# imaranresearch/LAMMPS-SPHERHARM

Measured on AMD Instinct MI355X. Metric: contact_pairs_per_sec, higher is better.
Workload: dtype f64; 1 GPU; BASELINE configs[1]: 100000 particles/GPU, 1 SH shape(s) L_max=6, dense packed bed (jittered HCP, spacing 1.9 mean radii), n_q=16 (Q=512 nodes/pair), pair_coeff kn=1000 exponent=1.25 (overlap volume + force + torque), inputs resident in HBM; particles_per_gpu=100000, lmax=6, nq=16, rule=sharp, backend=none, half_list_pairs_rank0=579574, contact_pairs_rank0=579574, touching_pairs_rank0=502600, contact_pairs_all_ranks=579574

## Files before the change

lammps-spherharm_amd/csrc/contact_kernel_azimuth.hpp:

```cpp
#pragma once
#include "contact_plan.hpp"
#include "jpoly.hpp"
#include "pair_params.hpp"
#include "pair_rotate.hpp"
#include "ring_tables.hpp"
#include "wave_ops.hpp"

namespace shp {


template <int L, bool NEEDV, int WPP = 1, bool SPEC = false>
__global__ void __launch_bounds__(64 * kMaxWavesPerBlock, SHP_JMIN_WAVES(L, NEEDV, WPP)) pair_contact_azimuth_kernel(const PairParams P)
{
  static_assert(L >= 0, "per-azimuth kernels: compiled orders only");
  constexpr int LJ = L;
  static_assert(!SPEC || (PairSpec<LJ>::nq > 0 && PairSpec<LJ>::wpp == WPP),
                "specialised instances: the orders PairSpec names");
  static_assert(WPP == 1 || WPP == 2, "one or two waves per pair");
  extern __shared__ __attribute__((aligned(16))) unsigned char smem_raw[];
  int lane = threadIdx.x & 63;
  const int wib = __builtin_amdgcn_readfirstlane((int)(threadIdx.x >> 6));
  const int w = P.slot0 + ((WPP == 2) ? (int)blockIdx.x : __builtin_amdgcn_readfirstlane((int)(blockIdx.x * P.waves_per_block)) + wib);
  const int half = (WPP == 2) ? wib : 0;
  const int tid = lane + 64 * half;
  constexpr int NT = 64 * WPP;
  if (w >= P.npairs) return;
  const int LL = L;
  typedef PairSpec<L> Spec;
  const int nq = SPEC ? Spec::nq : P.nq;
  const int P_ring_rows = SPEC ? Spec::rr : P.ring_rows;
  const int P_qcap = SPEC ? Spec::qc : P.qcap;
  constexpr bool P1S = SHP_SURFACE_PHASE1(L, NEEDV, WPP);
  constexpr bool CARRY = !P1S && SHP_CARRY_NODE(L, WPP);
  WaveLdsLayout W = (WPP == 2) ? pair_lds_layout2(LL, P_ring_rows, nq, P_qcap)
                               : wave_lds_layout(LL, P_ring_rows, false, nq, P_qcap);
  if constexpr (WPP == 2) {
    W.qri += half * W.qstride;
    W.qrj += half * W.qstride;
    W.qp += half * W.qstride;
    W.park += half * W.qstride;
  }
  typedef __attribute__((address_space(3))) unsigned char lds_byte_t;
  const unsigned wave_off = (WPP == 2) ? 0u : (unsigned)(wib * P.wave_lds_bytes);
  const unsigned wave_abs = __builtin_amdgcn_readfirstlane((unsigned)(size_t)(lds_byte_t*)smem_raw + wave_off);
#define WAVE_LDS() ((double*)(lds_byte_t*)(size_t)launder_s32(wave_abs))
  double* lw = WAVE_LDS();

  __builtin_amdgcn_s_setprio(3);
  const int* rid = P.rec_i + 4 * (size_t)w;
  constexpr int NSL = ((L + 1) * (L + 1) + NT - 1) / NT;
  double vi[NSL], vj[NSL];
  JPolyPre<LJ> pre;
  const double recv = P.rec[(size_t)kRecStride * w + (lane < kRecUsed ? lane : 0)];
  {
    constexpr int ns = (L + 1) * (L + 1);
#pragma unroll
    for (int t = 0; t < NSL; ++t) {
      const int e = tid + NT * t;
      const int ec = e < ns ? e : 0;
      if constexpr (rot_tiled(L)) {
        const int l = (int)__builtin_amdgcn_sqrtf((float)ec + 0.5f);
        const double* tile = P.rot + (size_t)((2 * w) >> 6) * rot_tile_doubles(L);
        const unsigned at = 64u * (unsigned)(l * l) + (unsigned)((2 * w) & 63) * (unsigned)(2 * l + 1) + (unsigned)(ec - l * l);
        vi[t] = tile[at];
        vj[t] = tile[at + (unsigned)(2 * l + 1)];
      } else {
        const size_t at = (size_t)(2 * w) * rot_row_doubles(L) + ec;
        vi[t] = P.rot[at];
        vj[t] = P.rot[at + rot_row_doubles(L)];
      }
    }
    pre.fetch(P, lane, nq);
  }
  double glt_first = 0.0, glw_first = 0.0;
  glw_first = P.glw[tid < nq ? tid : 0];
  if constexpr (L <= 8 && WPP == 1) {
    const int nr0 = P_ring_rows < nq ? P_ring_rows : nq;
    const int lg0 = ring_poly_map(nr0, L + 1, 64);
    const int kr = lg0 >= 1 ? (lane >> lg0) : lane / (L + 1);
    glt_first = P.glt[kr < nr0 ? kr : nr0 - 1];
  }
  const int status = rid[0];
  if (status == 0) return;
  double s_rho = 0.0, s_rj = 0.0, s_rj2 = 0.0, s_rho2 = 0.0, s_pj = 0.0, s_tol1 = 0.0, s_tol3 = 0.0, s_tiny = 0.0;
  {
    const cdptr rs = launder_uniform(P.rec + (size_t)kRecStride * w);
    s_rho = rs[FR_RHO];
    s_rj = rs[FR_RJ];
    s_rj2 = rs[FR_RJ2];
    s_rho2 = rs[FR_RHO2];
    s_pj = rs[FR_JPJ];
    s_tol1 = rs[FR_JTOL1];
    s_tol3 = rs[FR_JTOL3];
    s_tiny = rs[FR_JTINY];
  }
  const bool centre_in_bj = rid[3] != 0;
  if ((tid >= 12 && tid < 30) || (tid >= 36 && tid < kRecUsed)) lw[frj(tid)] = recv;
  if constexpr (L <= 8 && WPP == 1) lw[W.stash + lane] = glt_first;
#pragma unroll
  for (int t = 0; t < NSL; ++t)
    if (tid + NT * t < (LJ + 1) * (LJ + 1)) {
      lw[W.v0 + tid + NT * t] = vj[t];
      lw[W.v0i + tid + NT * t] = vi[t];
    }
  pair_sync<WPP>();
#if defined(SHP_ABL) && SHP_ABL == 1
  asm volatile("" ::"v"(lw[lane & 31]));
  return;
#endif
  jpoly_build<LJ, WPP>(P, lw, W, lane, nq, pre, glw_first, half);
#if defined(SHP_ABL) && SHP_ABL == 4
  asm volatile("" ::"v"(lw[W.pi + lane]));
  return;
#endif

  const double* fr = WAVE_LDS();

  bool centre_inside = false;
  if (NEEDV && centre_in_bj) {
    const double rho = fr[frj(FR_RHO)];
    const double rj = jpoly_eval<LJ>(fr + W.gh, -1.0, 0.0);
    centre_inside = (rho - rj <= 0.0);
  }

  const int npsi = 2 * nq;
  const unsigned magic = ((1u << 24) + (unsigned)npsi - 1u) / (unsigned)npsi;
  const int per_ring = nq / WPP;
  const unsigned magicr = ((1u << 24) + (unsigned)per_ring - 1u) / (unsigned)per_ring;
  const int nslabs = (nq * per_ring + 63) >> 6;
  const int rowlen = 4 * (LL + 1);

  {
    const int kend0 = (P_ring_rows < nq) ? P_ring_rows : nq;
    cap_frame_rings_poly<LJ, WPP>(P, WAVE_LDS(), W, lane, tid, 0, kend0, fr[frj(FR_HW)], fr[frj(FR_HM)], L <= 8 && WPP == 1);
  }
  bool first_group = true;
  double aV = 0.0, aS0 = 0.0, aS1 = 0.0, aS2 = 0.0, aT0 = 0.0, aT1 = 0.0, aT2 = 0.0;
#if defined(SHP_ABL) && SHP_ABL == 3
  int qhead = 0;
#endif
  int qcount = 0, slab = 0;

  while (slab < nslabs) {
  const int sfirst = slab;
  const int k0 = (int)(((unsigned)(sfirst << 6) * magicr) >> 24);
  const int kend = (k0 + P_ring_rows < nq) ? k0 + P_ring_rows : nq;
  const int slab_end = (kend == nq) ? nslabs : ((kend * per_ring) >> 6);
  if (slab_end <= slab) return;
  __builtin_amdgcn_s_setprio(3);
  {
    double* lr = WAVE_LDS();
    if (!first_group) {
      double* park = lr + W.park + lane;
      park[0] = aT2; park[64] = NEEDV ? aV : aS0;
      if constexpr (WPP == 2) __syncthreads();
      cap_frame_rings_poly<LJ, WPP>(P, lr, W, lane, tid, k0, kend - k0, lr[frj(FR_HW)], lr[frj(FR_HM)], false);
      park = WAVE_LDS() + W.park + lane;
      aT2 = park[0];
      if (NEEDV) aV = park[64]; else aS0 = park[64];
      wave_lds_sync();
    }
    first_group = false;
#if defined(SHP_ABL) && SHP_ABL == 2
    asm volatile("" ::"v"(lr[W.ring + lane]));
    return;
#endif
  }

  auto surface = [&](const double ri, const double rmu, const double rpsi, const double c, const double s, const double mu,
                     const double sig, const double isig, const double omi) __attribute__((always_inline)) {
    const double rad = ri * fma(ri, sig, rmu * sig * mu);
    const double tan_ = ri * rpsi * isig;
    const double A0 = fma(rad, c, tan_ * s);
    const double A1 = fma(rad, s, -tan_ * c);
    const double A2 = ri * fma(ri, mu, -(sig * sig) * rmu);
    aS0 = fma(omi, A0, aS0);
    aS1 = fma(omi, A1, aS1);
    aS2 = fma(omi, A2, aS2);
    const double wr = omi * ri;
    const double u0 = sig * c, u1 = sig * s;
    aT0 = fma(wr, u1 * A2 - mu * A1, aT0);
    aT1 = fma(wr, mu * A0 - u0 * A2, aT1);
    aT2 = fma(wr, u0 * A1 - u1 * A0, aT2);
  };
  auto phase2 = [&](auto dir_c, const int dp, const double dri, const double drj, const unsigned long long mdir)
                    __attribute__((always_inline)) {
    constexpr bool DIR = decltype(dir_c)::value;
    (void)dp; (void)dri; (void)drj; (void)mdir;
    wave_lds_sync();
    fr = WAVE_LDS();
    const int cnt = DIR ? 64 : (qcount < 64 ? qcount : 64);
    const bool active = DIR ? lane_of(mdir) : lane < cnt;
    if constexpr (!DIR) qcount -= cnt;
    const int e = DIR ? 0 : qcount + min(lane, cnt - 1);
#ifdef SHP_STATS
    if (lane == 0) atomicAdd(&P.dbg[4], 1ULL);
    if (active) atomicAdd(&P.dbg[7], 1ULL);
#endif
    int p;
    double ri;
    if constexpr (DIR) {
      p = dp;
      ri = dri;
    } else {
      p = ((const unsigned short*)(fr + W.qp))[e];
      ri = fr[W.qri + e];
    }
    int k = (int)(umul_sel<true>((unsigned)p, magic) >> 24);
    int l = p - mul_sel<true>(k, npsi);
    double omi = active ? fr[frj(FR_WSC)] * fr[W.glw + mul_sel<true>(k, jpoly_row(LJ))] : 0.0;
    const double omi3 = omi * (1.0 / 3.0);
    double c1 = 0.0, s1 = 0.0;
    if constexpr (!P1S) {
      c1 = P.cpsi[l];
      s1 = P.spsi[l];
    }
    double mu, sig;
    {
      const double* row = fr + W.ring + (k - k0) * rowlen;
      mu = row[1];
      sig = row[3];
    }

    double rin = 0.0;
    if (NEEDV) {
      const double rj0 = DIR ? drj : fr[W.qrj + e];
      double uj0, uj1;
      const int ghrow_ = W.gh + mul_sel<true>(l >= nq ? l - nq : l, jpoly_row(LJ));
      uj0 = mu;
      uj1 = (l >= nq) ? -sig : sig;
      double lo = 0.0, hi = ri, lam, xa = ri, ga, xb = ri, gb;
      {
        double bp, s2i;
        {
          const double rho = s_rho;
          bp = mu * rho;
          const double q0 = fma(ri, uj0, -rho), q1 = ri * uj1;
          s2i = fma(q0, q0, q1 * q1);
        }
        const double rho2l = s_rho2;
        if (!centre_in_bj) lo = bp - sqrt_nr1<true>(fma(bp, bp, -s_pj));
        lam = bp - sqrt_nr1<true>(fma(bp, bp, -(rho2l - rj0 * rj0)));
        if (!(lam > lo && lam < hi)) lam = 0.5 * (lo + hi);
        ga = gb = sqrt_nr1<true>(s2i) - rj0;
      }
      unsigned jrow_addr = wave_abs + 8u * (unsigned)ghrow_;
      unsigned long long mact;
      mact = centre_inside ? 0ULL : (DIR ? mdir : (cnt >= 64 ? ~0ULL : ((1ULL << cnt) - 1ULL)));
      auto iterate = [&](double& xa, double& ga, const double xb, const double gb, const double lam, double& gc,
                         const bool have3) __attribute__((always_inline)) {
#ifdef SHP_STATS
        if (lane == 0) atomicAdd(&P.dbg[5], 1ULL);
        if (lane_of(mact)) atomicAdd(&P.dbg[6], 1ULL);
#endif
        double y0, y1, ss2;
        y0 = fma(lam, uj0, -s_rho);
        y1 = lam * uj1;
        ss2 = fma(y0, y0, y1 * y1);
        const bool z0 = !(ss2 > 0.0);
        const double iv = rsqrt_nr1(ss2);
        double rj;
        jrow_addr = launder_u32(jrow_addr);
        rj = jpoly_eval<LJ>((const double*)(lds_byte_t*)(size_t)jrow_addr, y0 * iv, y1 * iv);
        const double Rjl = s_rj;
        double gl = ss2 * iv - rj;
        if (wave_any(z0)) {
          asm volatile("; rare: a point on x_j");
          gl = z0 ? -Rjl : gl;
        }
        {
          const bool pos = gl >= 0.0;
          lo = pos ? lam : lo;
          hi = pos ? hi : lam;
          const double dbl = gb - gl;
          double ext;
          if (!have3) {
            ext = fma(gl * (lam - xb), rcp_nr1(dbl), lam);
          } else {
            const double dab = ga - gb, dal = ga - gl;
            const double num = fma(xa * gb, gl * dbl, fma(lam * ga, gb * dab, -(xb * ga) * (gl * dal)));
            ext = num * rcp_nr1(dab * dal * dbl);
          }
          const bool inb = ext > lo && ext < hi;
          const bool accept = fabs(gl) <= (have3 ? s_tol3 : s_tol1);
          const bool tiny = hi - lo <= s_tiny;
          double res = ext, nxt = ext;
          unsigned long long mstop = wave_ballot(accept);
          if (mask_any(mact & (wave_ballot(tiny) | ~(wave_ballot(ext > lo) & wave_ballot(ext < hi))))) {
#ifdef SHP_STATS
            if (lane == 0) atomicAdd(&P.dbg[8], 1ULL);
#endif
            double sec = ext, e2 = ext;
            if (have3) {
              const double s2 = fma(gl * (lam - xb), rcp_nr1(dbl), lam);
              const bool fin0 = fabs(ext) <= 1e300;
              sec = (!fin0 || !inb) ? s2 : ext;
              e2 = fin0 ? ext : s2;
            }
            const double mid = 0.5 * (lo + hi);
            double n2 = (e2 > lo && e2 < hi) ? e2 : sec;
            n2 = (n2 > lo && n2 < hi) ? n2 : mid;
            const double accv = (fabs(e2) <= 1e300) ? fmin(fmax(e2, lo), hi) : lam;
            res = accept ? accv : (tiny ? mid : n2);
            nxt = n2;
            mstop |= wave_ballot(tiny);
          }
          rin = lane_of(mact) ? res : rin;
          mact &= ~mstop;
          gc = gl;
          xa = nxt;
        }
      };
      double gl0 = 0.0;
      if constexpr (SHP_PEEL(L)) {
      do {
        if (!mask_any(mact)) break;
        iterate(xa, ga, xb, gb, lam, gl0, false);
        if (!mask_any(mact)) break;
        iterate(xb, gb, lam, gl0, xa, ga, true);
        if (!mask_any(mact)) break;
        iterate(lam, gl0, xa, ga, xb, gb, true);
        for (int it = 3; it < 60; it = __builtin_amdgcn_readfirstlane(it + 3)) {
          if (!mask_any(mact)) break;
          iterate(xa, ga, xb, gb, lam, gl0, true);
          if (!mask_any(mact)) break;
          iterate(xb, gb, lam, gl0, xa, ga, true);
          if (!mask_any(mact)) break;
          iterate(lam, gl0, xa, ga, xb, gb, true);
        }
      } while (false);
      } else {
      for (int it = 0; it < 60; it = __builtin_amdgcn_readfirstlane(it + 3)) {
        if (!mask_any(mact)) break;
        iterate(xa, ga, xb, gb, lam, gl0, it >= 1);
        if (!mask_any(mact)) break;
        iterate(xb, gb, lam, gl0, xa, ga, true);
        if (!mask_any(mact)) break;
        iterate(lam, gl0, xa, ga, xb, gb, true);
      }
      }
      if constexpr (P1S) {
        if constexpr (!DIR) ri = fr[W.qri + (int)launder_u32((unsigned)e)];
        const double dv3 = ri * ri * ri - rin * rin * rin;
        aV = fma(omi3, dv3, aV);
      } else {
        auto ri_again = [&]() __attribute__((always_inline)) {
          const int lrow = l >= nq ? l - nq : l;
          const double* tgd = jpoly_trig_sep(LJ) ? fr + W.tr + 2 * lrow : fr + W.gh + mul_sel<true>(lrow, jpoly_row(LJ)) + jpoly_trig(LJ);
          double cd = 1.0, sd = 0.0;
          if constexpr (LJ >= 1) {
            const v2d csd = lds2(tgd);
            const double sgd = (l >= nq) ? -1.0 : 1.0;
            cd = sgd * csd[0];
            sd = sgd * csd[1];
          }
          return ring_value<LJ>(fr + W.ring + (k - k0) * rowlen, cd, sd);
        };
        if constexpr (!CARRY) {
          if constexpr (!DIR) {
            const int e2 = (int)launder_u32((unsigned)e);
            ri = fr[W.qri + e2];
            p = ((const unsigned short*)(fr + W.qp))[e2];
          }
          p = (int)launder_u32((unsigned)p);
          k = (int)(umul_sel<true>((unsigned)p, magic) >> 24);
          l = p - mul_sel<true>(k, npsi);
          omi = active ? fr[frj(FR_WSC)] * fr[W.glw + mul_sel<true>(k, jpoly_row(LJ))] : 0.0;
          const double* row = fr + W.ring + (k - k0) * rowlen;
          mu = row[1];
          sig = row[3];
          if constexpr (DIR) ri = ri_again();
        } else {
          if constexpr (DIR) {
            ri = ri_again();
          } else {
            const int e2 = (int)launder_u32((unsigned)e);
            ri = fr[W.qri + e2];
          }
        }
        const double dv3 = ri * ri * ri - rin * rin * rin;
        aV = fma(omi * (1.0 / 3.0), dv3, aV);
      }
    }

#if !(defined(SHP_ABL) && SHP_ABL == 6)
    if constexpr (!P1S) {
      fr = WAVE_LDS();
      double rmu, rpsi;
      const double sg = (l >= nq) ? -1.0 : 1.0;
      const int lrow = l >= nq ? l - nq : l;
      const double* tg = jpoly_trig_sep(LJ) ? fr + W.tr + 2 * lrow : fr + W.gh + mul_sel<true>(lrow, jpoly_row(LJ)) + jpoly_trig(LJ);
      if constexpr (LJ >= 1) {
        const v2d cs1 = lds2(tg);
        c1 = sg * cs1[0];
        s1 = sg * cs1[1];
      }
      ring_grad_rec<LJ>(fr + W.ring + (k - k0) * rowlen, c1, s1, rmu, rpsi);
      surface(ri, rmu, rpsi, c1, s1, mu, sig, rcp_nr1(sig), omi);
    }
#endif
    wave_lds_sync();
  };
  __builtin_amdgcn_s_setprio(0);
  for (;;) {
#define SHP_PUSH(m_, pn, rin_, rjn_)                                                                                  \
    {                                                                                                                  \
      if (m_ != 0ULL) {                                                                                                \
        if (lane_of(m_)) {                                                                                             \
          const int pos_ = qcount + (int)__builtin_amdgcn_mbcnt_hi((unsigned)(m_ >> 32),                               \
                                                    __builtin_amdgcn_mbcnt_lo((unsigned)m_, 0u));                      \
          double* lq_ = WAVE_LDS();                                                                                     \
          ((unsigned short*)(lq_ + W.qp))[pos_] = (unsigned short)(pn);                                                \
          lq_[W.qri + pos_] = (rin_);                                                                                  \
          lq_[W.qrj + pos_] = (rjn_);                                                                                  \
        }                                                                                                              \
        qcount += __builtin_popcountll(m_);                                                                            \
      }                                                                                                                \
    }
    while (qcount < 64 && slab < slab_end) {
      fr = WAVE_LDS();
      const int pp = (slab << 6) + lane;
      const int ppc = min(pp, nq * per_ring - 1);
      const int k = (int)(umul_sel<true>((unsigned)ppc, magicr) >> 24);
      const int l = ppc - mul_sel<true>(k, per_ring) + half * per_ring;
      const double* row = fr + W.ring + (k - k0) * rowlen;
      const v2d r01 = lds2(row);
      const double mu = r01[1], sig = row[3];
      const double* gr = fr + W.gh + mul_sel<true>(l, jpoly_row(LJ));
      double ria, rib;
      {
        double c1 = 1.0, s1 = 0.0, unused0, unused1;
        if constexpr (LJ >= 1) {
          const v2d cs1 = lds2(jpoly_trig_sep(LJ) ? fr + W.tr + 2 * l : gr + jpoly_trig(LJ));
          c1 = cs1[0];
          s1 = cs1[1];
        }
        ring_pair_rec<LJ, false>(row, r01[0], c1, s1, ria, rib, unused0, unused1);
      }
      const double rho = s_rho, rj2 = s_rj2;
      const double qa0 = fma(ria, mu, -rho), qa1 = ria * sig;
      const double qb0 = fma(rib, mu, -rho), qb1 = -rib * sig;
      const double sa2 = fma(qa0, qa0, qa1 * qa1), sb2 = fma(qb0, qb0, qb1 * qb1);
      const int nvalid = nq * per_ring - (slab << 6);
      const unsigned long long mvalid = nvalid >= 64 ? ~0ULL : ((1ULL << nvalid) - 1ULL);
      const unsigned long long mca = wave_ballot(sa2 < rj2) & mvalid, mcb = wave_ballot(sb2 < rj2) & mvalid;
      if ((mca | mcb) == 0ULL) {
#ifdef SHP_STATS
        if (lane == 0) atomicAdd(&P.dbg[0], 2ULL);
#endif
        ++slab;
        continue;
      }
      const bool za = !(sa2 > 0.0), zb = !(sb2 > 0.0);
      const unsigned long long mza = wave_ballot(za), mzb = wave_ballot(zb);
      const double inva = rsqrt_nr1(sa2), invb = rsqrt_nr1(sb2);
      double rjae, rjbe;
      jpoly_eval2<LJ>(fr + W.gh + mul_sel<true>(l, jpoly_row(LJ)), qa0 * inva, qa1 * inva, qb0 * invb, qb1 * invb, rjae, rjbe);
      const double Rjl = s_rj;
      double rja = rjae, rjb = rjbe;
      if (mask_any(mza | mzb)) {
        asm volatile("; rare: a node on x_j");
        rja = za ? Rjl : rjae;
        rjb = zb ? Rjl : rjbe;
      }
      const unsigned long long ma = mca & (mza | wave_ballot(sa2 * inva < rja));
      const unsigned long long mb = mcb & (mzb | wave_ballot(sb2 * invb < rjb));
#if !(defined(SHP_ABL) && SHP_ABL == 6)
      if (P1S && (ma | mb) != 0ULL) {
        static_assert(!P1S || LJ >= 1, "the trig of the first order comes from particle j's table");
        const double* fg = WAVE_LDS();
        const double* rowg = fg + W.ring + (k - k0) * rowlen;
        const v2d cs1 = lds2(jpoly_trig_sep(LJ) ? fg + W.tr + 2 * l : fg + W.gh + mul_sel<true>(l, jpoly_row(LJ)) + jpoly_trig(LJ));
        const double c1 = cs1[0], s1 = cs1[1];
        const v2d g23 = lds2(rowg + 2);
        const double mug = rowg[1], sigg = g23[1];
        double rmua, rmub, rpsia, rpsib;
        ring_pair_rec<LJ, true, SHP_GRAD_CHUNK(L)>(rowg, g23[0], c1, s1, rmua, rmub, rpsia, rpsib);
        const double om = fg[frj(FR_WSC)] * fg[W.glw + mul_sel<true>(k, jpoly_row(LJ))];
        const double isig = rcp_nr1(sigg);
        surface(ria, rmua, rpsia, c1, s1, mug, sigg, isig, lane_of(ma) ? om : 0.0);
        surface(rib, rmub, rpsib, -c1, -s1, mug, sigg, isig, lane_of(mb) ? om : 0.0);
      }
#endif
      if constexpr (P1S && !NEEDV) {
#ifdef SHP_STATS
        if (lane == 0) atomicAdd(&P.dbg[0], 2ULL);
        if (lane_of(mca)) atomicAdd(&P.dbg[1], 1ULL);
        if (lane_of(mcb)) atomicAdd(&P.dbg[1], 1ULL);
        if (lane == 0) atomicAdd(&P.dbg[2], 2ULL);
        if (lane_of(ma)) atomicAdd(&P.dbg[3], 1ULL);
        if (lane_of(mb)) atomicAdd(&P.dbg[3], 1ULL);
#endif
        ++slab;
        continue;
      }
      const int pa = mul_sel<true>(k, npsi) + l;
#ifdef SHP_STATS
      if (qcount + __builtin_popcountll(ma) + __builtin_popcountll(mb) > W.qcap) {
        if (lane == 0) atomicAdd(&P.dbg[9], 1ULL);
      }
#endif
      if (qcount + __builtin_popcountll(ma) + __builtin_popcountll(mb) > W.qcap) {
        const unsigned long long mboth = ma & mb;
        SHP_PUSH(mboth, pa, ria, rja);
        const bool second = lane_of(mb);
        ++slab;
#ifdef SHP_STATS
        if (lane == 0) atomicAdd(&P.dbg[0], 2ULL);
        if (lane_of(mca)) atomicAdd(&P.dbg[1], 1ULL);
        if (lane_of(mcb)) atomicAdd(&P.dbg[1], 1ULL);
        if (lane == 0) atomicAdd(&P.dbg[2], 2ULL);
        if (lane_of(ma)) atomicAdd(&P.dbg[3], 1ULL);
        if (lane_of(mb)) atomicAdd(&P.dbg[3], 1ULL);
        if (lane == 0) atomicAdd(&P.dbg[10], 1ULL);
        if (lane == 0 && P.dbg[15]) atomicAdd(&P.dbg[64 + w], (unsigned long long)(__builtin_popcountll(ma) + __builtin_popcountll(mb)));
#endif
        phase2(BoolC<true>{}, second ? pa + nq : pa, second ? rib : ria, second ? rjb : rja, ma | mb);
        continue;
      }
#ifdef SHP_STATS
      if (lane == 0) atomicAdd(&P.dbg[0], 2ULL);
      if (lane_of(mca)) atomicAdd(&P.dbg[1], 1ULL);
      if (lane_of(mcb)) atomicAdd(&P.dbg[1], 1ULL);
      if (lane == 0) atomicAdd(&P.dbg[2], 2ULL);
      if (lane_of(ma)) atomicAdd(&P.dbg[3], 1ULL);
      if (lane_of(mb)) atomicAdd(&P.dbg[3], 1ULL);
      if (lane == 0 && P.dbg[15]) atomicAdd(&P.dbg[64 + w], (unsigned long long)(__builtin_popcountll(ma) + __builtin_popcountll(mb)));
#endif
      ++slab;
      SHP_PUSH(ma, pa, ria, rja);
      SHP_PUSH(mb, pa + nq, rib, rjb);
    }
#undef SHP_PUSH
    if ((P1S && !NEEDV) || qcount == 0) break;
#if defined(SHP_ABL) && SHP_ABL == 3
    qhead = (qhead + qcount) & (kQueue - 1);
    qcount = 0;
    continue;
#endif

    phase2(BoolC<false>{}, 0, 0.0, 0.0, 0ULL);
  }
  }

  __builtin_amdgcn_s_setprio(3);
  lane = fresh_lane();
  if constexpr (WPP == 2) __syncthreads();
  {
    double* red = WAVE_LDS() + ((WPP == 2 && half) ? (int)(P.wave_lds_bytes >> 3) - kRedPerWave : kFrameJ);
    red[0 * kRedStride + lane] = aS0; red[1 * kRedStride + lane] = aS1; red[2 * kRedStride + lane] = aS2;
    red[3 * kRedStride + lane] = aT0; red[4 * kRedStride + lane] = aT1; red[5 * kRedStride + lane] = aT2;
    red[6 * kRedStride + lane] = NEEDV ? aV : 0.0;
    wave_lds_sync();
    double* part = red + 7 * kRedStride;
    if (lane < 56) {
      const double* src = red + (lane >> 3) * kRedStride + (lane & 7);
      part[lane] = ((src[0] + src[8]) + (src[16] + src[24])) + ((src[32] + src[40]) + (src[48] + src[56]));
    }
    wave_lds_sync();
    double* tot = part + 56;
    if (lane < 7) {
      const double* src = part + 8 * lane;
      tot[lane] = ((src[0] + src[1]) + (src[2] + src[3])) + ((src[4] + src[5]) + (src[6] + src[7]));
    }
    wave_lds_sync();
    if constexpr (WPP == 2) {
      __syncthreads();
      if (half != 0) return;
      if (lane < 7) tot[lane] += WAVE_LDS()[(int)(P.wave_lds_bytes >> 3) - kRedPerWave + 7 * kRedStride + 56 + lane];
      wave_lds_sync();
    }
  }
  if (lane >= 6) return;
  fr = WAVE_LDS();
  const double* tot = fr + kFrameJ + 7 * kRedStride + 56;
  double* fcomp = (double*)tot + 7;
  const int comp = (lane >= 3) ? lane - 3 : lane;
  const bool is_t = lane >= 3;
  const double a0 = tot[is_t ? 3 : 0], a1 = tot[is_t ? 4 : 1], a2 = tot[is_t ? 5 : 2];
  const double val = fr[frj(FR_E1) + comp] * a0 + fr[frj(FR_E2) + comp] * a1 + fr[frj(FR_C) + comp] * a2;
  const double aVt = tot[6];

  LateParams& E = *late_params();
  if (E.pair_out) {
    double* o = E.pair_out + 7 * (size_t)w;
    o[1 + lane] = val;
    if (lane == 0) o[0] = aVt;
  }
  const bool touched = NEEDV ? (aVt > 0.0) : (wave_ballot(!is_t && val != 0.0) != 0ULL);
  if (E.flags && lane == 0) E.flags[w] = touched ? 2 : 1;
  if (!touched) return;

  const int* ij = (const int*)(fr + frj(FR_IJ));
  const int i = ij[0], j = ij[1];
  const double knij = fr[frj(FR_KN)], mij = fr[frj(FR_EXPO)];
  const double vm1 = (mij == 1.0) ? 1.0 : pow_quarter(aVt, mij - 1.0);
  const double pn = knij * mij * vm1;
  const double Fm = -pn * val;
  fcomp[lane] = Fm;
  wave_lds_sync();
  double* const det = E.pair_ft;
  if (det) det[12 * (size_t)w + lane] = Fm;
  else atomicAdd((is_t ? E.torque : E.f) + 3 * (size_t)i + comp, Fm);
  const bool applyj = E.newton_pair || j < E.nlocal;
  if (applyj) {
    const int c1 = (comp == 2) ? 0 : comp + 1, c2 = (comp == 0) ? 2 : comp - 1;
    double vj = -Fm;
    if (is_t) vj -= fr[frj(FR_D) + c1] * (-fcomp[c2]) - fr[frj(FR_D) + c2] * (-fcomp[c1]);
    if (det) det[12 * (size_t)w + 6 + lane] = vj;
    else atomicAdd((is_t ? E.torque : E.f) + 3 * (size_t)j + comp, vj);
  }
  if ((E.eflag || E.vflag) && E.pair_ev) {
    const double share = E.newton_pair ? 1.0 : (0.5 + (j < E.nlocal ? 0.5 : 0.0));
    double* row = E.pair_ev + 8 * (size_t)w;
    if (E.vflag) {
      const int a = (lane < 3) ? lane : ((lane == 5) ? 1 : 0);
      const int b = (lane < 3) ? lane : ((lane == 3) ? 1 : 2);
      row[1 + lane] = share * (-fr[frj(FR_D) + a]) * fcomp[b];
    }
    if (E.eflag && lane == 0) row[0] = share * knij * (vm1 * aVt);
  }
  if (lane != 0) return;
  if (E.eatom || E.vatom) {
    const double F0 = fcomp[0], F1 = fcomp[1], F2 = fcomp[2];
    const double d0 = fr[frj(FR_D)], d1 = fr[frj(FR_D) + 1], d2 = fr[frj(FR_D) + 2];
    const bool owni = E.newton_pair || i < E.nlocal;
    if (E.eatom) {
      const double eh = 0.5 * knij * (vm1 * aVt);
      if (owni) atomicAdd(&E.eatom[i], eh);
      if (applyj) atomicAdd(&E.eatom[j], eh);
    }
    if (E.vatom) {
      const double v[6] = {0.5 * (-d0) * F0, 0.5 * (-d1) * F1, 0.5 * (-d2) * F2,
                           0.5 * (-d0) * F1, 0.5 * (-d0) * F2, 0.5 * (-d1) * F2};
      for (int a = 0; a < 6; ++a) {
        if (owni) atomicAdd(&E.vatom[6 * (size_t)i + a], v[a]);
        if (applyj) atomicAdd(&E.vatom[6 * (size_t)j + a], v[a]);
      }
    }
  }
}
#undef WAVE_LDS

}
```

lammps-spherharm_amd/csrc/pair_kernel.hpp:

```cpp
#pragma once
#include "contact_plan.hpp"
#include "pair_params.hpp"
#include "pair_rotate.hpp"

#ifndef SHP_WMIN_WAVES
#define SHP_WMIN_WAVES(L) (((L) >= 0 && (L) <= 6 && (L) != 3) ? 5 : 4)
#endif
#ifndef SHP_MIN_WAVES
#define SHP_MIN_WAVES(L, NEEDV) \
  ((NEEDV) ? (((L) == 0 || (L) == 1 || (L) == 6) ? 6 : 5) : (((L) >= 0 && (L) <= 6) ? 6 : 5))
#endif
#ifndef SHP_JMIN_WAVES
#define SHP_JMIN_WAVES(L, NEEDV, WPP) (((L) <= 4) ? 6 : (((L) <= 6 || ((L) == 9 && (WPP) == 1 && !(NEEDV))) ? 5 : 4))
#endif

#ifndef SHP_PEEL
#define SHP_PEEL(L) ((L) >= 6)
#endif
#ifndef SHP_CARRY_NODE
#define SHP_CARRY_NODE(L, WPP) ((L) >= 6 && !((L) == 9 && (WPP) == 1))
#endif
#ifndef SHP_SURFACE_PHASE1
#define SHP_SURFACE_PHASE1(L, NEEDV, WPP) ((L) >= 6 && !((L) == 12 && (WPP) == 2))
#endif
#ifndef SHP_GRAD_CHUNK
#define SHP_GRAD_CHUNK(L) ((L) >= 7 ? 1 : 0)
#endif

namespace shp {
template <bool B>
struct BoolC { static constexpr bool value = B; };
}

#include "contact_kernel_azimuth.hpp"
#include "contact_kernel_body.hpp"

namespace shp {

template <int L, bool AZIMUTH = false, int WPP = 1, bool SPEC = false>
const void* contact_kernel(const bool needv)
{
  if constexpr (AZIMUTH)
    return needv ? (const void*)pair_contact_azimuth_kernel<L, true, WPP, SPEC>
                 : (const void*)pair_contact_azimuth_kernel<L, false, WPP, SPEC>;
  else
    return needv ? (const void*)pair_contact_body_kernel<L, true>
                 : (const void*)pair_contact_body_kernel<L, false>;
}
template <int L>
const void* pair_contact_instance(const ContactPlan& p, const bool needv)
{
  if constexpr (L >= 0) {
    if (p.weighted) return (const void*)pair_contact_body_kernel<L, true, true>;
    if constexpr (PairSpec<L>::nq > 0)
      if (p.spec) return contact_kernel<L, true, PairSpec<L>::wpp, true>(needv);
    if constexpr (split_compiled(L))
      if (p.waves_per_pair == 2) return contact_kernel<L, true, 2>(needv);
    if (p.family == 1) return contact_kernel<L, true>(needv);
  }
  return contact_kernel<L>(needv);
}

template <int L>
void launch_pair_contact(const PairParams& P, const ContactPlan& plan, bool needv, hipStream_t st, hipEvent_t wait_before_contact)
{
  const int nslots = P.npairs - P.slot0;
  if (nslots <= 0) return;
  if constexpr (L >= 0) {
    if (plan.family == 1)
      hipLaunchKernelGGL((pair_rotate_lane_kernel<L>), dim3((2 * (unsigned)nslots + 63) / 64), dim3(64),
                         RotLaneLds<L>::bytes(), st, P, const_cast<double*>(P.rot));
  }
  if (wait_before_contact) (void)hipStreamWaitEvent(st, wait_before_contact, 0);
  const int wpb = plan.waves_per_block;
  const size_t lds = (size_t)wpb * plan.lds_bytes;
  const void* kern = pair_contact_instance<L>(plan, needv);
  if (lds > 65536) (void)hipFuncSetAttribute(kern, hipFuncAttributeMaxDynamicSharedMemorySize, (int)lds);
  void* args[] = {const_cast<PairParams*>(&P)};
  (void)hipLaunchKernel(kern, dim3((nslots + wpb - 1) / wpb), dim3(64 * wpb * plan.waves_per_pair), args, lds, st);
}

}
```

lammps-spherharm_amd/csrc/ring_tables.hpp:

```cpp
#pragma once
#include "contact_plan.hpp"
#include "sh_const.hpp"
#include "wave_ops.hpp"

namespace shp {

template <int L, int WPP, bool DENSE>
__device__ __forceinline__ void ring_lane_map(const int lane, const int nrows, int& krl, int& g, int& G, int& rpc, int& lg)
{
  const int lg1 = (nrows <= 8) ? 3 : (nrows <= 16) ? 2 : (nrows <= 32) ? 1 : 0;
  lg = lg1 + (WPP == 2 ? 1 : 0);
  G = 1 << lg;
  krl = lane >> lg;
  g = lane & (G - 1);
  rpc = (64 * WPP) >> lg;
  if constexpr (DENSE && L >= 1 && WPP == 1) {
    if ((L + 1) * nrows <= 64) {
      G = L + 1;
      krl = lane / (L + 1);
      g = lane - krl * (L + 1);
      rpc = 64 / (L + 1);
      lg = 0;
    }
  }
}

template <int L, bool PRE = false, int WPP = 1, bool DENSE = false>
__device__ __forceinline__ void cap_frame_rings(const PairParams& P, double* __restrict__ lw, const WaveLdsLayout& W,
                                                const int LL, const int lane, const int k0, const int nrows,
                                                const double hw, const double hm, const bool have_first = false)
{
  const double* ch = lw + W.v0;
  double* ring = lw + W.ring;
  int krl, g, G, rpc, lg;
  ring_lane_map<L, WPP, DENSE>(lane, nrows, krl, g, G, rpc, lg);
  for (int kr0 = 0; kr0 < nrows; kr0 += rpc) {
    const int kr = kr0 + krl;
    const bool row_ok = kr < nrows && krl < rpc;
    const double tk = (PRE && have_first && k0 == 0 && kr0 == 0) ? lw[W.stash + lane] : P.glt[k0 + (row_ok ? kr : 0)];
    const double mu = fma(hw, tk, hm);
    const double sig2 = fmax(0.0, fma(-mu, mu, 1.0));
    const double sig = sqrt_nr(sig2);
    double sp = 1.0, sigG = sig;
    for (int t = 0; t < G - 1; ++t) {
      if (t < g) sp *= sig;
    }
    for (int t = 0; t < lg; ++t) sigG *= sigG;
    for (int m0 = 0; m0 <= LL; m0 += G) {
      const int m = m0 + g;
      const bool ok = row_ok && m <= LL;
      const int mc = ok ? m : 0;
      const double* rcm = P.rc + (sh_moff(LL, mc) - mc);
      const double* cp = ch + mc;
      const double* cm = ch - mc;
      const bool modd = (mc & 1) != 0;
      double qe = modd ? 0.0 : 1.0, qo = modd ? 1.0 : 0.0, de = 0.0, dd = 0.0;
      double wa = cp[mc * mc + mc], wb = cm[mc * mc + mc], wad = 0.0, wbd = 0.0;
      constexpr int NPRE = (PRE && L >= 1) ? L : 1;
      double pa[NPRE];
      if constexpr (PRE && L >= 1) {
#pragma unroll
        for (int n = 1; n <= L; ++n) {
          if (n <= m0) continue;
          pa[n - 1] = rcm[n];
        }
#pragma unroll
        for (int n = 1; n <= L; ++n) {
          if (n <= m0) continue;
          asm volatile("" : "+v"(pa[n - 1]));
        }
      }
#pragma unroll
      for (int n = 1; n <= ((L >= 0) ? L : LL); ++n) {
        if (n <= m0) continue;
        if (ok && n > m) {
          const double a = (PRE && L >= 1) ? pa[(PRE && L >= 1) ? n - 1 : 0] : rcm[n];
          const double ca = cp[n * n + n], cbm = cm[n * n + n];
          if (n & 1) {
            dd = fma(a, fma(mu, de, qe), -dd);
            qo = fma(a, mu * qe, -qo);
            wa = fma(ca, qo, wa); wb = fma(cbm, qo, wb); wad = fma(ca, dd, wad); wbd = fma(cbm, dd, wbd);
          } else {
            de = fma(a, fma(mu, dd, qo), -de);
            qe = fma(a, mu * qo, -qe);
            wa = fma(ca, qe, wa); wb = fma(cbm, qe, wb); wad = fma(ca, de, wad); wbd = fma(cbm, de, wbd);
          }
        }
      }
      if (ok) {
        const double f = (m > 0) ? (double)m * mu * rcp_nr(sig2) : 0.0;
        double* o = ring + 4 * (kr * (LL + 1) + m);
        o[0] = sp * wa;
        o[2] = sp * fma(-f, wa, wad);
        if (m == 0) {
          o[1] = mu;
          o[3] = sig;
        } else {
          o[1] = sp * wb;
          o[3] = sp * fma(-f, wb, wbd);
        }
      }
      sp *= sigG;
    }
  }
  pair_sync<WPP>();
}

__host__ __device__ inline int ring_poly_map(const int nrows, const int K, const int NT)
{
  const int nent = nrows * K;
  if (nent <= NT) return -1;
  int lg = 0;
  while ((NT >> (lg + 1)) >= nrows && (1 << lg) < K) ++lg;
  if (lg < 1) return -1;
  const int E = (K + (1 << lg) - 1) >> lg, passes = (nent + NT - 1) / NT;
  return (25 + 44 * E < 69 * passes) ? lg : -1;
}

template <int L, int WPP, class PP = PairParams>
__device__ __forceinline__ void cap_frame_rings_poly(const PP& P, double* __restrict__ lw, const WaveLdsLayout& W,
                                                     const int lane, const int tid, const int k0, const int nrows,
                                                     const double hw, const double hm, const bool have_first)
{
  constexpr int K = L + 1, NT = 64 * WPP;
  const double* pi = lw + W.pi;
  double* ring = lw + W.ring;
  const int nent = nrows * K;
  const int lg = ring_poly_map(nrows, K, NT);
  auto entry = [&](const int m, const int e, const bool store, const double mu, const double sig, const double isig)
                   __attribute__((always_inline)) {
    const double* row = pi + (2 * K) * m;
    v2d c[K];
#pragma unroll
    for (int t = 0; t < K; ++t) c[t] = lds2(row + 2 * t);
#define SHP_EL(j) c[(j) >> 1][(j) & 1]
    double pc = SHP_EL(L), ps = SHP_EL(K + L), dc = 0.0, ds = 0.0;
    if constexpr (L >= 1) {
      dc = pc;
      ds = ps;
      pc = fma(pc, mu, SHP_EL(L - 1));
      ps = fma(ps, mu, SHP_EL(K + L - 1));
#pragma unroll
      for (int q = L - 2; q >= 0; --q) {
        dc = fma(dc, mu, pc);
        ds = fma(ds, mu, ps);
        pc = fma(pc, mu, SHP_EL(q));
        ps = fma(ps, mu, SHP_EL(K + q));
      }
    }
#undef SHP_EL
    const bool odd = (m & 1) != 0;
    const double sm = odd ? sig : 1.0;
    const double tm = odd ? -mu * isig : 0.0;
    const double A = sm * pc, dA = fma(tm, pc, sm * dc);
    double B = sm * ps, dB = fma(tm, ps, sm * ds);
    if (m == 0) {
      B = mu;
      dB = sig;
    }
    if (store) {
      double* o = ring + 4 * e;
      *(v2d*)__builtin_assume_aligned(o, 16) = v2d{A, B};
      *(v2d*)__builtin_assume_aligned(o + 2, 16) = v2d{dA, dB};
    }
  };
  if (lg >= 1) {
    const int G = 1 << lg, kr = tid >> lg, g = tid & (G - 1);
    const int krc = min(kr, nrows - 1);
    const double tk = (have_first && k0 == 0) ? lw[W.stash + lane] : P.glt[k0 + krc];
    const double mu = fma(hw, tk, hm);
    const double sig2 = max_raw(fma(-mu, mu, 1.0), 1e-300);
    const double isig = rsqrt_nr(sig2);
    const double sig = sig2 * isig;
    for (int m0 = 0; m0 < K; m0 += G) {
      const int m = m0 + g;
      entry(min(m, K - 1), krc * K + m, kr < nrows && m < K, mu, sig, isig);
    }
  } else {
    for (int e0 = 0; e0 < nent; e0 += NT) {
      const int e = e0 + tid;
      const int ec = min(e, nent - 1);
      const int kr = (int)((unsigned)ec / (unsigned)K), m = ec - kr * K;
      const double tk = (have_first && k0 == 0 && e0 == 0) ? lw[W.stash + lane] : P.glt[k0 + kr];
      const double mu = fma(hw, tk, hm);
      const double sig2 = max_raw(fma(-mu, mu, 1.0), 1e-300);
      const double isig = rsqrt_nr(sig2);
      const double sig = sig2 * isig;
      entry(m, e, e < nent, mu, sig, isig);
    }
  }
  pair_sync<WPP>();
}

__host__ __device__ constexpr bool trig_lmajor(int L) { return L >= 2 && L <= 6; }

struct QuadLayout {
  int lmax, npsi, nm;
  size_t glt, glw, cpsi, spsi, trig, trigj, size;
  int trig_stride;
  QuadLayout(const int L, const int nq)
      : lmax(L), npsi(2 * nq), nm(L >= 2 ? L - 1 : 0), glt(0), glw(nq), cpsi(2 * (size_t)nq), spsi(4 * (size_t)nq),
        trig(6 * (size_t)nq), trigj(trig + (size_t)nm * 2 * npsi), size(trigj + (size_t)nq * (L + 2) * 2),
        trig_stride(trig_lmajor(L) ? 2 * (L - 1) : 4 * nq)
  {
  }
  size_t trig_at(const int l, const int m) const
  {
    return trig + 2 * (trig_lmajor(lmax) ? ((size_t)l * nm + (m - 2)) : ((size_t)(m - 2) * npsi + l));
  }
  size_t trigj_at(const int l, const int m) const { return trigj + ((size_t)l * (lmax + 2) + m) * 2; }
};

template <int L, bool GRAD>
__device__ __forceinline__ void ring_eval(const double* __restrict__ row, const int LL, const double c1, const double s1,
                                          const double* __restrict__ tr, const int tstride, double& r, double& rmu,
                                          double& rpsi)
{
  r = row[0];
  rmu = GRAD ? row[2] : 0.0;
  rpsi = 0.0;
  double cm = c1, sm = s1;
  const int lim = (L >= 0) ? L : LL;
#pragma unroll
  for (int m = 1; m <= lim; ++m) {
    if (L >= 2 && m >= 2) {
      cm = tr[trig_lmajor(L) ? 2 * (m - 2) : (m - 2) * tstride];
      sm = tr[(trig_lmajor(L) ? 2 * (m - 2) : (m - 2) * tstride) + 1];
    }
    const v2d ab = lds2(row + 4 * m);
    const double A = ab[0], B = ab[1];
    r = fma(A, cm, r);
    r = fma(B, sm, r);
    if (GRAD) {
      const v2d dab = lds2(row + 4 * m + 2);
      rmu = fma(dab[0], cm, rmu);
      rmu = fma(dab[1], sm, rmu);
      const double dm = (double)m;
      rpsi = fma(dm * B, cm, rpsi);
      rpsi = fma(-dm * A, sm, rpsi);
    }
    if (L < 2 && m < lim) {
      const double c = fma(cm, c1, -(sm * s1)), s = fma(cm, s1, sm * c1);
      cm = c;
      sm = s;
    }
  }
}

template <int L, bool GRAD, int CHUNK = 0>
__device__ __forceinline__ void ring_pair_rec(const double* __restrict__ row0, const double a0, const double c1, const double s1,
                                              double& va, double& vb, double& wa, double& wb)
{
  double ve = a0, vo = 0.0, we = 0.0, wo = 0.0;
  const double* row = row0;
  if constexpr (L >= 1) {
    double cm = c1, sm = s1, cp = 1.0, sp = 0.0;
    const double tc = c1 + c1;
#pragma unroll
    for (int m = 1; m <= L; ++m) {
      const v2d ab = lds2(row + 4 * m);
      const double A = ab[0], B = ab[1];
      if constexpr (!GRAD) {
        if (m & 1) vo = fma(A, cm, fma(B, sm, vo));
        else ve = fma(A, cm, fma(B, sm, ve));
      } else {
        const v2d dab = lds2(row + 4 * m + 2);
        const double t = fma(B, cm, -(A * sm)), dm = (double)m;
        if (m & 1) {
          vo = fma(dab[0], cm, fma(dab[1], sm, vo));
          wo = (m == 1) ? t : fma(dm, t, wo);
        } else {
          ve = fma(dab[0], cm, fma(dab[1], sm, ve));
          we = (m == 2) ? dm * t : fma(dm, t, we);
        }
      }
      if (m < L) {
        const double c = fma(tc, cm, -cp), s = fma(tc, sm, -sp);
        cp = cm;
        sp = sm;
        cm = c;
        sm = s;
        if constexpr (GRAD && CHUNK > 0) {
          if (m % CHUNK == 0) {
            unsigned ra_ = (unsigned)(size_t)(const __attribute__((address_space(3))) double*)row;
            asm volatile("" : "+v"(ra_), "+v"(ve), "+v"(vo), "+v"(cm), "+v"(sm));
            row = (const double*)(const __attribute__((address_space(3))) double*)(size_t)ra_;
          }
        }
      }
    }
  }
  va = ve + vo;
  vb = ve - vo;
  wa = we + wo;
  wb = we - wo;
}

}
```

Baseline: 279.3 million contact-pairs/s.

## Evaluate azimuth nodes in symmetric quads for L=6 phase-1 surface pass

Adds a quad path to the specialised L=6 single-wave no-volume azimuth kernel. Each lane now handles four nodes related by psi reflection and mirroring. One Fourier recurrence split into even and odd cosine and sine sums gives all four radii and gradients, so each lane covers half as many ring positions. The goal is to cut trig recurrence and LDS row loads per node. The cost is more code, more register pressure, and two node_pair evaluations per lane.

```diff
diff --git a/lammps-spherharm_amd/csrc/azimuth_quads.hpp b/lammps-spherharm_amd/csrc/azimuth_quads.hpp
--- /dev/null
+++ b/lammps-spherharm_amd/csrc/azimuth_quads.hpp
@@ -0,0 +1,48 @@
+#pragma once
+#include "sh_const.hpp"
+
+namespace shp {
+
+struct QuadSums {
+  double ce, co, se, so;
+};
+
+SHP_HD constexpr int quad_reflected_row(const int l, const int nq) { return nq - 1 - l; }
+SHP_HD constexpr int quad_mirror(const int l, const int nq) { return 2 * nq - 1 - l; }
+SHP_HD constexpr bool quad_rule(const int nq) { return nq >= 4 && 64 % (2 * nq) == 0; }
+
+SHP_HD inline void quad_add(QuadSums& q, const int m, const double a, const double b, const double cm, const double sm)
+{
+  if (m & 1) {
+    q.co = __builtin_fma(a, cm, q.co);
+    q.so = __builtin_fma(b, sm, q.so);
+  } else {
+    q.ce = __builtin_fma(a, cm, q.ce);
+    q.se = __builtin_fma(b, sm, q.se);
+  }
+}
+SHP_HD inline void quad_add_dpsi(QuadSums& q, const int m, const double A, const double B, const double cm, const double sm)
+{
+  const double dm = (double)m;
+  quad_add(q, m, B, -A, dm * cm, dm * sm);
+}
+SHP_HD inline void quad_trig_next(const double tc, double& cm, double& sm, double& cp, double& sp)
+{
+  const double c = __builtin_fma(tc, cm, -cp), s = __builtin_fma(tc, sm, -sp);
+  cp = cm;
+  sp = sm;
+  cm = c;
+  sm = s;
+}
+SHP_HD inline void quad_pair0(const QuadSums& q, double& f0, double& f1)
+{
+  f0 = (q.ce + q.co) + (q.se + q.so);
+  f1 = (q.ce - q.co) + (q.se - q.so);
+}
+SHP_HD inline void quad_pair1(const QuadSums& q, double& f2, double& f3)
+{
+  f2 = (q.ce - q.co) - (q.se - q.so);
+  f3 = (q.ce + q.co) - (q.se + q.so);
+}
+
+}
diff --git a/lammps-spherharm_amd/csrc/contact_kernel_azimuth.hpp b/lammps-spherharm_amd/csrc/contact_kernel_azimuth.hpp
--- a/lammps-spherharm_amd/csrc/contact_kernel_azimuth.hpp
+++ b/lammps-spherharm_amd/csrc/contact_kernel_azimuth.hpp
@@ -125,7 +125,10 @@
 
   const int npsi = 2 * nq;
   const unsigned magic = ((1u << 24) + (unsigned)npsi - 1u) / (unsigned)npsi;
-  const int per_ring = nq / WPP;
+  constexpr bool QP = SPEC && !NEEDV && P1S && SHP_PHASE1_QUADS(L, NEEDV, WPP);
+  static_assert(!QP || (quad_rule(Spec::nq) && Spec::rr == Spec::nq), "quads: whole rings per slab, one ring group");
+  constexpr bool quads = QP;
+  const int per_ring = quads ? nq / 2 : nq / WPP;
   const unsigned magicr = ((1u << 24) + (unsigned)per_ring - 1u) / (unsigned)per_ring;
   const int nslabs = (nq * per_ring + 63) >> 6;
   const int rowlen = 4 * (LL + 1);
@@ -418,6 +421,111 @@
       }                                                                                                                \
     }
     while (qcount < 64 && slab < slab_end) {
+      if constexpr (QP) {
+      if (quads) {
+        fr = WAVE_LDS();
+        const int nquads = nq * per_ring;
+        const int ppc = min((slab << 6) + lane, nquads - 1);
+        const int k = (int)(umul_sel<true>((unsigned)ppc, magicr) >> 24);
+        const int l = ppc - mul_sel<true>(k, per_ring);
+        const int l2 = quad_reflected_row(l, nq);
+        const double* row = fr + W.ring + (k - k0) * rowlen;
+        const v2d r01 = lds2(row);
+        const double mu = r01[1], sig = row[3];
+        double ria, rib, ric, rid;
+        {
+          const v2d cs1 = lds2(jpoly_trig_sep(LJ) ? fr + W.tr + 2 * l : fr + W.gh + mul_sel<true>(l, jpoly_row(LJ)) + jpoly_trig(LJ));
+          QuadSums qv, unused;
+          ring_quad_rec<LJ, false>(row, r01[0], cs1[0], cs1[1], qv, unused);
+          quad_pair0(qv, ria, rib);
+          quad_pair1(qv, ric, rid);
+        }
+        const int nvalid = nquads - (slab << 6);
+        const unsigned long long mvalid = nvalid >= 64 ? ~0ULL : ((1ULL << nvalid) - 1ULL);
+        auto node_pair = [&](const int lr, const double ra, const double rb, unsigned long long& ma, unsigned long long& mb,
+                             unsigned long long& mca, unsigned long long& mcb) __attribute__((always_inline)) {
+          double rja, rjb;
+          const double rho = s_rho, rj2 = s_rj2;
+          const double qa0 = fma(ra, mu, -rho), qa1 = ra * sig;
+          const double qb0 = fma(rb, mu, -rho), qb1 = -rb * sig;
+          const double sa2 = fma(qa0, qa0, qa1 * qa1), sb2 = fma(qb0, qb0, qb1 * qb1);
+          mca = wave_ballot(sa2 < rj2) & mvalid;
+          mcb = wave_ballot(sb2 < rj2) & mvalid;
+          ma = mb = 0ULL;
+          if ((mca | mcb) == 0ULL) return;
+          const bool za = !(sa2 > 0.0), zb = !(sb2 > 0.0);
+          const unsigned long long mza = wave_ballot(za), mzb = wave_ballot(zb);
+          const double inva = rsqrt_nr1(sa2), invb = rsqrt_nr1(sb2);
+          double rjae, rjbe;
+          jpoly_eval2<LJ>(WAVE_LDS() + W.gh + mul_sel<true>(lr, jpoly_row(LJ)), qa0 * inva, qa1 * inva, qb0 * invb, qb1 * invb, rjae, rjbe);
+          rja = rjae;
+          rjb = rjbe;
+          if (mask_any(mza | mzb)) {
+            asm volatile("; rare: a node on x_j");
+            rja = za ? s_rj : rjae;
+            rjb = zb ? s_rj : rjbe;
+          }
+          ma = mca & (mza | wave_ballot(sa2 * inva < rja));
+          mb = mcb & (mzb | wave_ballot(sb2 * invb < rjb));
+        };
+        {
+          unsigned long long ma, mb, mc, md, mca, mcb, mcc, mcd;
+          node_pair(l, ria, rib, ma, mb, mca, mcb);
+          asm volatile("" : "+v"(ric), "+v"(rid));
+          node_pair(l2, ric, rid, mc, md, mcc, mcd);
+#ifdef SHP_STATS
+          if (lane == 0) atomicAdd(&P.dbg[0], 4ULL);
+          if (lane_of(mca)) atomicAdd(&P.dbg[1], 1ULL);
+          if (lane_of(mcb)) atomicAdd(&P.dbg[1], 1ULL);
+          if (lane_of(mcc)) atomicAdd(&P.dbg[1], 1ULL);
+          if (lane_of(mcd)) atomicAdd(&P.dbg[1], 1ULL);
+          if (lane == 0 && (mca | mcb) != 0ULL) atomicAdd(&P.dbg[2], 2ULL);
+          if (lane == 0 && (mcc | mcd) != 0ULL) atomicAdd(&P.dbg[2], 2ULL);
+          if (lane_of(ma)) atomicAdd(&P.dbg[3], 1ULL);
+          if (lane_of(mb)) atomicAdd(&P.dbg[3], 1ULL);
+          if (lane_of(mc)) atomicAdd(&P.dbg[3], 1ULL);
+          if (lane_of(md)) atomicAdd(&P.dbg[3], 1ULL);
+#endif
+          if ((ma | mb | mc | md) == 0ULL) {
+            ++slab;
+            continue;
+          }
+#ifdef SHP_STATS
+          if (lane == 0 && P.dbg[15])
+            atomicAdd(&P.dbg[64 + w], (unsigned long long)(__builtin_popcountll(ma) + __builtin_popcountll(mb) + __builtin_popcountll(mc) + __builtin_popcountll(md)));
+#endif
+#if !(defined(SHP_ABL) && SHP_ABL == 6)
+          {
+            const double* fg = WAVE_LDS();
+            const double* rowg = fg + W.ring + (k - k0) * rowlen;
+            const v2d cs1 = lds2(jpoly_trig_sep(LJ) ? fg + W.tr + 2 * l : fg + W.gh + mul_sel<true>(l, jpoly_row(LJ)) + jpoly_trig(LJ));
+            const double c1 = cs1[0], s1 = cs1[1];
+            const v2d g23 = lds2(rowg + 2);
+            const double mug = rowg[1], sigg = g23[1];
+            QuadSums qm, qs;
+            ring_quad_rec<LJ, true>(rowg, g23[0], c1, s1, qm, qs);
+            const double om = fg[frj(FR_WSC)] * fg[W.glw + mul_sel<true>(k, jpoly_row(LJ))];
+            const double isig = rcp_nr1(sigg);
+            double rmu0, rmu1, rpsi0, rpsi1;
+            if ((ma | mb) != 0ULL) {
+              quad_pair0(qm, rmu0, rmu1);
+              quad_pair0(qs, rpsi0, rpsi1);
+              surface(ria, rmu0, rpsi0, c1, s1, mug, sigg, isig, lane_of(ma) ? om : 0.0);
+              surface(rib, rmu1, rpsi1, -c1, -s1, mug, sigg, isig, lane_of(mb) ? om : 0.0);
+            }
+            if ((mc | md) != 0ULL) {
+              quad_pair1(qm, rmu0, rmu1);
+              quad_pair1(qs, rpsi0, rpsi1);
+              surface(ric, rmu0, rpsi0, -c1, s1, mug, sigg, isig, lane_of(mc) ? om : 0.0);
+              surface(rid, rmu1, rpsi1, c1, -s1, mug, sigg, isig, lane_of(md) ? om : 0.0);
+            }
+          }
+#endif
+        }
+        ++slab;
+        continue;
+      }
+      }
       fr = WAVE_LDS();
       const int pp = (slab << 6) + lane;
       const int ppc = min(pp, nq * per_ring - 1);
diff --git a/lammps-spherharm_amd/csrc/pair_kernel.hpp b/lammps-spherharm_amd/csrc/pair_kernel.hpp
--- a/lammps-spherharm_amd/csrc/pair_kernel.hpp
+++ b/lammps-spherharm_amd/csrc/pair_kernel.hpp
@@ -22,6 +22,9 @@
 #endif
 #ifndef SHP_SURFACE_PHASE1
 #define SHP_SURFACE_PHASE1(L, NEEDV, WPP) ((L) >= 6 && !((L) == 12 && (WPP) == 2))
+#endif
+#ifndef SHP_PHASE1_QUADS
+#define SHP_PHASE1_QUADS(L, NEEDV, WPP) ((L) == 6 && (WPP) == 1 && !(NEEDV) && SHP_SURFACE_PHASE1(L, NEEDV, WPP))
 #endif
 #ifndef SHP_GRAD_CHUNK
 #define SHP_GRAD_CHUNK(L) ((L) >= 7 ? 1 : 0)
diff --git a/lammps-spherharm_amd/csrc/ring_tables.hpp b/lammps-spherharm_amd/csrc/ring_tables.hpp
--- a/lammps-spherharm_amd/csrc/ring_tables.hpp
+++ b/lammps-spherharm_amd/csrc/ring_tables.hpp
@@ -1,4 +1,5 @@
 #pragma once
+#include "azimuth_quads.hpp"
 #include "contact_plan.hpp"
 #include "sh_const.hpp"
 #include "wave_ops.hpp"
@@ -296,4 +297,28 @@
   wb = we - wo;
 }
 
-}
+template <int L, bool GRAD>
+__device__ __forceinline__ void ring_quad_rec(const double* __restrict__ row, const double a0, const double c1, const double s1,
+                                              QuadSums& v, QuadSums& w)
+{
+  v = QuadSums{a0, 0.0, 0.0, 0.0};
+  w = QuadSums{0.0, 0.0, 0.0, 0.0};
+  if constexpr (L >= 1) {
+    double cm = c1, sm = s1, cp = 1.0, sp = 0.0;
+    const double tc = c1 + c1;
+#pragma unroll
+    for (int m = 1; m <= L; ++m) {
+      const v2d ab = lds2(row + 4 * m);
+      if constexpr (!GRAD) {
+        quad_add(v, m, ab[0], ab[1], cm, sm);
+      } else {
+        const v2d dab = lds2(row + 4 * m + 2);
+        quad_add(v, m, dab[0], dab[1], cm, sm);
+        quad_add_dpsi(w, m, ab[0], ab[1], cm, sm);
+      }
+      if (m < L) quad_trig_next(tc, cm, sm, cp, sp);
+    }
+  }
+}
+
+}
```

Result: slower. 275.4 million contact-pairs/s (-1.4%).
